# chaeyeongyun/VQ_SEG

Hardware: AMD Instinct MI355X
Metric: train images/sec @512x512 vqreptunet1x1 K=512 (higher is better)
Workload: dtype bf16; 1 GPU; CPS training iteration (2 x vqreptunet1x1, ResNet-50 encoder, K=[0,0,512,512,512], v1 recipe: 6 forwards + 4 backwards + 2 Adam steps) on 512x512x3 images -- BASELINE configs[2] (the metric's configuration): vqreptunet1x1 512x512, K = 512; labelled_per_gpu=32, unlabelled_per_gpu=32, parallelism=dp1, collectives=none (one process), conv_dtype=bf16

## Files before the change

include/vqseg.h:

```cpp
#ifndef VQSEG_H
#define VQSEG_H

#include <stddef.h>
#include <stdint.h>

#ifdef __cplusplus
extern "C" {
#endif

#define VQSEG_ABI_VERSION 1

#define VQSEG_EINVAL  (-1)
#define VQSEG_ENOSPC  (-2)
#define VQSEG_ENODEV  (-3)

int         vqseg_abi_version(void);
const char* vqseg_last_error(void);
const char* vqseg_kernel_name(const char* entry_point);

int vqseg_set_option(const char* key, int value);

int vqseg_profile_begin(int capacity);
int vqseg_profile_collect(int max_records, int64_t* n_rows_host, int* channels_host,
                          int* n_codes_host, float* ms_host,
// ... 52 lines not shown
int vqseg_kmeans_finalize_f32(const float* sums, const int64_t* counts, float* means,
                              int channels, int n_codes, void* stream);


int vqseg_vq_code_sums(int bf16, const void* x, const int64_t* idx, int64_t n_rows, int channels, int n_codes,
                       float* sums, int64_t* counts, void* workspace, size_t workspace_bytes, void* stream);
int vqseg_vq_ema_update_f32(float* cluster_size, float* embed_avg, float* codebook, const float* sums,
                            const int64_t* counts, int channels, int n_codes, float decay, float eps, float* scratch,
                            void* stream);
int vqseg_vq_revive_candidates(int bf16, const void* x, int64_t n_rows, int channels, int n_codes, uint64_t seed,
                               const int64_t* counter, int rank, int world, float* cand, float* ok, void* stream);
int vqseg_vq_ema_update_revive_f32(float* cluster_size, float* embed_avg, float* codebook, const float* sums,
                                   const int64_t* counts, int channels, int n_codes, float decay, float eps, float* scratch,
                                   const float* cand, const float* ok, float threshold, int64_t* counter, int64_t* revived,
                                   void* stream);


size_t vqseg_conv_packed_elems(int cout, int cin, int kh, int kw, int transpose_flip);
int vqseg_conv_pack_weights_f32(const float* w, int cout, int cin, int kh, int kw, int transpose_flip,
                                void* hi, void* lo, void* stream);

int64_t vqseg_conv_stat_slots(int64_t m_rows, int cout);
int vqseg_conv2d_f(const void* x, const void* x2, int c1, const void* w_hi, const void* w_lo, void* y,
                   float* stat_partial, int n, int h, int w, int cin, int cout, int kh, int kw, int stride,
                   int pad, int reflect, int up, int ho, int wo, int precise, void* stream);

int vqseg_conv2d_affine_f(const void* x, const void* x2, int c1, const void* w_hi, const void* w_lo,
                          const float* scale, const float* shift, const void* res, int relu, void* y,
                          int n, int h, int w, int cin, int cout, int kh, int kw, int stride, int pad, int reflect,
                          int ho, int wo, int precise, void* stream);
int vqseg_conv2d_affine_bits_f(const void* x, const void* w_hi, const float* scale, const float* shift, const void* res,
                               const unsigned char* res_bits, void* y, int n, int h, int w, int cin, int cout, int kh, int kw,
                               int pad, int ho, int wo, void* stream);

size_t vqseg_conv2d_wgrad_workspace_bytes(int n, int h, int w, int cin, int ho, int wo, int cout, int kh, int kw);
int vqseg_conv2d_wgrad_f(const void* gy, const void* x, const void* x2, int c1, int n, int h, int w, int cin,
                         int ho, int wo, int cout, int kh, int kw, int stride, int pad, int reflect, int precise,
                         int cin_out, int im2col, int accumulate, void* workspace, size_t workspace_bytes, float* gw,
                         void* stream);
int vqseg_conv2d_wgrad2_f(const void* gy, const void* x, const void* x2, int n, const void* gy_b, const void* x_b, const void* x2_b,
                          int n_b, int c1, int h, int w, int cin, int ho, int wo, int cout, int kh, int kw, int stride, int pad,
                          int reflect, int precise, int cin_out, int im2col, int accumulate, void* workspace, size_t workspace_bytes,
                          float* gw, void* stream);

int vqseg_bn_sync_ints(int c);
int vqseg_bn_finalize_f(float* partial, int64_t m_rows, int c, const float* gamma, const float* beta,
                        float* run_mean, float* run_var, float momentum, float eps, int training,
                        float* scale, float* shift, float* save_mean, float* save_invstd,
                        int64_t* num_batches_tracked , int* sync, void* stream);
int vqseg_bn_apply_f(int bf16, const void* y, const void* res, const float* scale, const float* shift,
                     int64_t m_rows, int c, int relu, void* out, void* stream);
size_t vqseg_bn_backward_workspace_floats(int64_t m_rows, int c);
int vqseg_bn_backward_f(int bf16, const void* g_out, const void* out, const void* y, const float* mean,
                        const float* invstd, const float* gamma, const float* fwd_scale, const float* fwd_shift,
                        int64_t m_rows, int c, int relu, int training, int accumulate,
                        float* workspace, float* dgamma, float* dbeta, void* g_y, void* g_res, int* sync, void* stream);
int vqseg_bn_apply_bits_f(const void* y, const void* res, const float* scale, const float* shift, int64_t m_rows, int c,
                          void* out, unsigned char* bits, void* stream);
int vqseg_bn_backward_bits_f(const void* g_out, const unsigned char* bits, const void* y, const float* mean,
                             const float* invstd, const float* gamma, int64_t m_rows, int c, int training, int accumulate,
                             float* workspace, float* dgamma, float* dbeta, void* g_y, void* g_res, int* sync, void* stream);

int vqseg_maxpool3x3s2_f(int bf16, int backward, const void* x, const void* g, int n, int h, int w, int c,
                         void* out, unsigned char* idx, void* stream);

int vqseg_bilinear_f(int bf16, int backward, const void* src, int n, int h, int w, int c, int ho, int wo,
// ... 123 lines not shown
```

vq_seg_amd/_hip.py:

```python
from __future__ import annotations

import ctypes
import os
from ctypes import c_char_p, c_double, c_float, c_int, c_int64, c_size_t, c_void_p
from typing import Optional, Tuple

import numpy as np
import torch

_HERE = os.path.dirname(os.path.abspath(__file__))
LIB_PATH = os.environ.get("VQSEG_LIB") or os.path.join(_HERE, "libvqseg_hip.so")

SYMBOLS = {
    "vqseg_abi_version": (c_int, []),
    "vqseg_last_error": (c_char_p, []),
    "vqseg_kernel_name": (c_char_p, [c_char_p]),
    "vqseg_set_option": (c_int, [c_char_p, c_int]),
    "vqseg_profile_begin": (c_int, [c_int]),
    "vqseg_profile_collect": (c_int, [c_int, c_void_p, c_void_p, c_void_p, c_void_p, c_void_p]),
    "vqseg_conv_profile_begin": (c_int, [c_int]),
    "vqseg_conv_profile_collect": (c_int, [c_int, c_void_p, c_void_p, c_void_p, c_void_p]),
    "vqseg_vq_workspace_bytes": (c_size_t, [c_int64, c_int, c_int]),
    "vqseg_vq_filter_counter_offset": (c_size_t, [c_int64, c_int, c_int]),
    "vqseg_vq_tiles_per_wave": (c_int, [c_int, c_void_p, c_void_p]),
    "vqseg_vq_forward_f32": (c_int, [c_void_p, c_void_p, c_void_p, c_int64, c_int, c_int, c_int, c_float, c_void_p,
                                     c_void_p, c_void_p, c_void_p, c_void_p, c_void_p, c_size_t, c_void_p]),
    "vqseg_vq_forward_bf16": (c_int, [c_void_p, c_void_p, c_void_p, c_int64, c_int, c_int, c_int, c_float, c_void_p,
                                      c_void_p, c_void_p, c_void_p, c_void_p, c_void_p, c_size_t, c_void_p]),
    "vqseg_vq_forward_group": (c_int, [c_int, c_int] + [c_void_p] * 6 + [c_int, c_void_p] + [c_void_p] * 6 + [c_void_p]),
    "vqseg_vq_backward_bf16": (c_int, [c_void_p, c_void_p, c_void_p, c_void_p, c_void_p, c_int64, c_int, c_float, c_void_p, c_void_p]),
    "vqseg_vq_assign_f32": (c_int, [c_void_p, c_void_p, c_void_p, c_int64, c_int, c_int, c_void_p, c_void_p, c_void_p,
                                    c_size_t, c_void_p]),
    "vqseg_vq_assign_bf16": (c_int, [c_void_p, c_void_p, c_void_p, c_int64, c_int, c_int, c_void_p, c_void_p, c_void_p,
                                     c_size_t, c_void_p]),
    "vqseg_vq_prepared_bytes": (c_size_t, [c_int, c_int]),
    "vqseg_vq_prepare_f32": (c_int, [c_void_p, c_int, c_int, c_void_p, c_size_t, c_void_p]),
    "vqseg_vq_backward_f32": (c_int, [c_void_p, c_void_p, c_void_p, c_void_p, c_int64, c_int, c_float, c_void_p,
                                      c_void_p]),
    "vqseg_kmeans_workspace_bytes": (c_size_t, [c_int64, c_int, c_int]),
    "vqseg_kmeans_f32": (c_int, [c_void_p, c_void_p, c_void_p, c_int64, c_int, c_int, c_int, c_void_p, c_size_t,
                                 c_void_p]),
    "vqseg_kmeans_accumulate_f32": (c_int, [c_void_p, c_void_p, c_int64, c_int, c_int, c_void_p, c_void_p, c_void_p,
                                            c_size_t, c_void_p]),
    "vqseg_kmeans_finalize_f32": (c_int, [c_void_p, c_void_p, c_void_p, c_int, c_int, c_void_p]),
    "vqseg_vq_code_sums": (c_int, [c_int, c_void_p, c_void_p, c_int64, c_int, c_int, c_void_p, c_void_p, c_void_p, c_size_t, c_void_p]),
    "vqseg_vq_ema_update_f32": (c_int, [c_void_p, c_void_p, c_void_p, c_void_p, c_void_p, c_int, c_int, c_float, c_float, c_void_p,
                                        c_void_p]),
    "vqseg_vq_revive_candidates": (c_int, [c_int, c_void_p, c_int64, c_int, c_int, ctypes.c_uint64, c_void_p, c_int, c_int, c_void_p, c_void_p,
                                           c_void_p]),
    "vqseg_vq_ema_update_revive_f32": (c_int, [c_void_p, c_void_p, c_void_p, c_void_p, c_void_p, c_int, c_int, c_float, c_float, c_void_p,
                                               c_void_p, c_void_p, c_float, c_void_p, c_void_p, c_void_p]),
    "vqseg_conv_packed_elems": (c_size_t, [c_int] * 5),
    "vqseg_conv_pack_weights_f32": (c_int, [c_void_p] + [c_int] * 5 + [c_void_p, c_void_p, c_void_p]),
    "vqseg_conv_stat_slots": (c_int64, [c_int64, c_int]),
    "vqseg_conv2d_f": (c_int, [c_void_p, c_void_p, c_int, c_void_p, c_void_p, c_void_p, c_void_p] + [c_int] * 14 + [c_void_p]),
    "vqseg_conv2d_affine_f": (c_int, [c_void_p, c_void_p, c_int, c_void_p, c_void_p, c_void_p, c_void_p, c_void_p, c_int, c_void_p] +
                              [c_int] * 13 + [c_void_p]),
    "vqseg_conv2d_wgrad_workspace_bytes": (c_size_t, [c_int] * 9),
    "vqseg_conv2d_wgrad_f": (c_int, [c_void_p, c_void_p, c_void_p] + [c_int] * 17 + [c_void_p, c_size_t, c_void_p, c_void_p]),
    "vqseg_conv2d_wgrad2_f": (c_int, [c_void_p, c_void_p, c_void_p, c_int, c_void_p, c_void_p, c_void_p, c_int] + [c_int] * 16 +
                              [c_void_p, c_size_t, c_void_p, c_void_p]),
    "vqseg_bn_sync_ints": (c_int, [c_int]),
    "vqseg_bn_finalize_f": (c_int, [c_void_p, c_int64, c_int, c_void_p, c_void_p, c_void_p, c_void_p, c_float, c_float, c_int,
                                   c_void_p, c_void_p, c_void_p, c_void_p, c_void_p, c_void_p, c_void_p]),
    "vqseg_bn_apply_f": (c_int, [c_int, c_void_p, c_void_p, c_void_p, c_void_p, c_int64, c_int, c_int, c_void_p, c_void_p]),
    "vqseg_bn_backward_workspace_floats": (c_size_t, [c_int64, c_int]),
    "vqseg_bn_backward_f": (c_int, [c_int] + [c_void_p] * 8 + [c_int64, c_int, c_int, c_int, c_int] + [c_void_p] * 7),
    "vqseg_conv2d_affine_bits_f": (c_int, [c_void_p] * 7 + [c_int] * 10 + [c_void_p]),
    "vqseg_bn_apply_bits_f": (c_int, [c_void_p] * 4 + [c_int64, c_int, c_void_p, c_void_p, c_void_p]),
    "vqseg_bn_backward_bits_f": (c_int, [c_void_p] * 6 + [c_int64, c_int, c_int, c_int] + [c_void_p] * 7),
    "vqseg_maxpool3x3s2_f": (c_int, [c_int, c_int, c_void_p, c_void_p, c_int, c_int, c_int, c_int, c_void_p, c_void_p, c_void_p]),
    "vqseg_bilinear_f": (c_int, [c_int, c_int, c_void_p] + [c_int] * 7 + [c_void_p, c_void_p]),
    "vqseg_head1x1_forward_f": (c_int, [c_int, c_void_p, c_void_p, c_int64, c_int, c_int, c_void_p, c_void_p]),
    "vqseg_head1x1_backward_workspace_floats": (c_size_t, [c_int64, c_int, c_int]),
    "vqseg_head1x1_backward_f": (c_int, [c_int, c_void_p, c_void_p, c_void_p, c_int64, c_int, c_int, c_void_p, c_void_p,
                                        c_void_p, c_void_p]),
    "vqseg_proto_loss_workspace_bytes": (c_size_t, [c_int64, c_int, c_int]),
    "vqseg_proto_loss_forward_f": (c_int, [c_int, c_void_p, c_void_p, c_void_p, c_void_p, c_void_p, c_int64, c_int, c_int, c_int,
                                           c_float, c_float, c_int, c_void_p, c_size_t, c_void_p, c_void_p]),
    "vqseg_proto_loss_backward_f": (c_int, [c_int, c_void_p, c_void_p, c_void_p, c_void_p, c_void_p, c_int64, c_int, c_int, c_int,
                                            c_float, c_float, c_int, c_void_p, c_void_p, c_void_p, c_void_p, c_size_t, c_void_p]),
    "vqseg_dice_workspace_bytes": (c_size_t, [c_int, c_int, c_int64]),
    "vqseg_dice_sums_forward_f": (c_int, [c_void_p, c_int64, c_int64, c_int64, c_void_p, c_int, c_int, c_int64, c_int64, c_void_p, c_size_t,
                                          c_void_p, c_void_p, c_void_p]),
    "vqseg_dice_sums_backward_f": (c_int, [c_void_p, c_int64, c_int64, c_int64, c_void_p, c_int, c_int, c_int64, c_int64, c_void_p,
                                           c_void_p, c_void_p, c_void_p]),
    "vqseg_dice_ce_sums_forward_f": (c_int, [c_void_p, c_int64, c_int64, c_int64, c_void_p, c_int, c_int, c_int64, c_int64, c_void_p,
                                             c_size_t, c_void_p, c_void_p, c_void_p, c_void_p]),
    "vqseg_dice_ce_sums_backward_f": (c_int, [c_void_p, c_int64, c_int64, c_int64, c_void_p, c_int, c_int, c_int64, c_int64, c_void_p,
                                              c_void_p, c_void_p, c_void_p, c_void_p]),
# ... 482 lines not shown
```

vq_seg_amd/csrc/conv_kernels.h:

```cpp
#pragma once
#include <hip/hip_runtime.h>
#include <stddef.h>
#include <stdint.h>

namespace vqseg {

struct ConvArgs {
    const void* x;
    const void* x2;
    int C1;
    const unsigned short* w_hi;
    const unsigned short* w_lo;
    void* y;
    float* stat_partial;
    int N, H, W, Cin, Ho, Wo, Cout, KH, KW, stride, pad, reflect, up;
    const float* ep_scale;
    const float* ep_shift;
    const void* ep_res;
    int ep_relu;
    int pair_chunks = 0, pair_tiles = 0;
    int out_s3 = 0;
    int s3_in = 0, s3_cs1 = 0, s3_cs2 = 0;
    int pad_w = -1;
    int omap = 0, omap_h = 0, omap_w = 0, omap_ph = 0, omap_pw = 0;
// ... 21 lines not shown
    int per_tap_only;
    const void* gy_b = nullptr;
    const void* x_b = nullptr;
    const void* x2_b = nullptr;
    int Na = 0;
    int xcd_slabs = 0;
};

hipError_t launch_conv(const ConvArgs& a, int precise, hipStream_t st);
long dgrad_s2_fold_rows(int N, int H, int W, int reflect);
hipError_t launch_dgrad_s2_fold(const void* gy, const unsigned short* w_hi, void* gx, int N, int Ho, int Wo, int Cout, int Cin, int H, int W,
                                int reflect, hipStream_t st);
hipError_t launch_stem7_fused(const float* x, const unsigned short* w_img, void* y, float* stat_partial, const float* ep_scale, const float* ep_shift,
                              int relu, int N, int H, int W, int reflect, int s3, hipStream_t st);
hipError_t conv_profile_begin(int capacity);
void conv_profile_release();
int conv_profile_collect(int max_records, double* flops, int* kind, float* ms, int* shape);
int conv_set_option(const char* key, int value);
int wgrad_slabs(const WgradArgs& a, int precise);
int wgrad_slabs_max(const WgradArgs& a);
hipError_t launch_wgrad(const WgradArgs& a, int precise, int slabs, int* final_layout, hipStream_t st);
hipError_t launch_wgrad_reduce(const float* partial, int slabs, int Cout, int Cin, int Cin_out, int KH, int KW, int im2col, int accumulate,
                               float* gw, hipStream_t st);
size_t packed_elems(int Cout, int Cin, int KH, int KW, int transpose_flip);
hipError_t launch_pack_weights(const float* w, int Cout, int Cin, int KH, int KW, int transpose_flip, unsigned short* hi,
                               unsigned short* lo, hipStream_t st);
hipError_t launch_pack_all(const float* w, int Cout, int Cin, int K, int C1, unsigned short* fwd, unsigned short* tr, unsigned short* s3,
                           hipStream_t st);
hipError_t launch_pack_weights_s2(const float* w, int Cout, int Cin, int K, unsigned short* hi, unsigned short* lo, hipStream_t st);
hipError_t launch_dgrad_s2(const void* gy, const unsigned short* w_hi, const unsigned short* w_lo, void* gx, int N, int Ho, int Wo,
                           int Cout, int Cin, int K, int OH, int OW, int precise, int accumulate, hipStream_t st);
hipError_t launch_reflect_ring(const void* gy, const unsigned short* t_hi, void* ring, int N, int H, int W, int Cgy, int Cgx, hipStream_t st);
hipError_t launch_pack_weights_s3(const float* w, int Cout, int Cin, int C1, int KH, int KW, unsigned short* out, hipStream_t st);

}
```

vq_seg_amd/csrc/nn_abi.hip:

```cpp
#include <hip/hip_runtime.h>
#include <stdarg.h>
#include <stdio.h>
#include <string.h>

#include "../../include/vqseg.h"
#include "conv_kernels.h"
#include "vq_kernels.h"
#include "nn_kernels.h"
#include "loss_kernels.h"
#include <math.h>

extern "C" int vqseg_set_error(int code, const char* msg);

namespace {
int bad(const char* msg) { return vqseg_set_error(VQSEG_EINVAL, msg); }
int hipfail(hipError_t e, const char* where) {
    char buf[256];
    snprintf(buf, sizeof(buf), "%s: %s", where, hipGetErrorString(e));
    return vqseg_set_error((int)e, buf);
}
bool a16(const void* p) { return (reinterpret_cast<uintptr_t>(p) & 15u) == 0; }

int conv_rows_per_slot(int cout) { return cout >= 64 ? 64 : 32; }
}
// ... 55 lines not shown
                          int kw, int stride, int pad, int reflect, int ho, int wo, int precise, void* stream) {
    if (!scale || !shift) return bad("conv2d_affine: null scale / shift");
    if (res && !a16(res)) return bad("conv2d_affine: pointers must be 16-byte aligned");
    if (precise == 2) {
        if (cin % 32 || cout % 8 || c1 % 32 || c1 <= 0 || c1 > cin) return bad("conv2d_affine (split-3): needs Cin, C1 % 32 == 0 and Cout % 8 == 0");
        if (!x || !w_hi || !y || (c1 < cin && !x2)) return bad("conv2d: null pointer");
        if (n <= 0 || h <= 0 || w <= 0 || ho <= 0 || wo <= 0 || kh <= 0 || kw <= 0 || stride <= 0) return bad("conv2d: non-positive dimension");
        if (!a16(x) || !a16(x2) || !a16(w_hi) || !a16(y)) return bad("conv2d: pointers must be 16-byte aligned");
        if (reflect && (pad >= h || pad >= w)) return bad("conv2d: reflect padding needs pad < size");
        vqseg::ConvArgs a;
        a.x = x; a.x2 = x2; a.C1 = 3 * c1;
        a.w_hi = static_cast<const unsigned short*>(w_hi); a.w_lo = nullptr;
        a.y = y; a.stat_partial = nullptr;
        a.N = n; a.H = h; a.W = w; a.Cin = 3 * cin; a.Ho = ho; a.Wo = wo; a.Cout = cout; a.KH = kh; a.KW = kw;
        a.stride = stride; a.pad = pad; a.reflect = reflect; a.up = 1;
        a.ep_scale = scale; a.ep_shift = shift; a.ep_res = res; a.ep_relu = relu;
        a.out_s3 = 1;
        a.s3_in = 1; a.s3_cs1 = c1; a.s3_cs2 = cin - c1;
        hipError_t e = vqseg::launch_conv(a, 0, static_cast<hipStream_t>(stream));
        return e == hipSuccess ? 0 : hipfail(e, "conv kernel (split-3)");
    }
    return conv2d_impl(x, x2, c1, w_hi, w_lo, y, nullptr, scale, shift, res, relu, n, h, w, cin, cout, kh, kw, stride, pad, reflect, 1,
                       ho, wo, precise, stream);
}

int vqseg_conv2d_affine_bits_f(const void* x, const void* w_hi, const float* scale, const float* shift, const void* res,
                               const unsigned char* res_bits, void* y, int n, int h, int w, int cin, int cout, int kh, int kw, int pad,
                               int ho, int wo, void* stream) {
    if (!scale || !shift || !res || !res_bits) return bad("conv2d_affine_bits: null pointer");
    if (!a16(res)) return bad("conv2d_affine_bits: pointers must be 16-byte aligned");
    if (cout % 8) return bad("conv2d_affine_bits: Cout must be a multiple of 8");
    return conv2d_impl(x, nullptr, cin, w_hi, nullptr, y, nullptr, scale, shift, res, 0, n, h, w, cin, cout, kh, kw, 1, pad, 0, 1, ho, wo, 0,
                       stream, res_bits);
}

int vqseg_conv_profile_begin(int capacity) {
    if (capacity <= 0 || capacity > (1 << 20)) return bad("conv_profile_begin: capacity out of range");
    hipError_t e = vqseg::conv_profile_begin(capacity);
    return e == hipSuccess ? 0 : hipfail(e, "conv_profile_begin");
}

int vqseg_conv_profile_collect(int max_records, double* flops_host, int* kind_host, float* ms_host, int* shape_host) {
    if (max_records <= 0 || !flops_host || !kind_host || !ms_host) return bad("conv_profile_collect: bad argument");
    return vqseg::conv_profile_collect(max_records, flops_host, kind_host, ms_host, shape_host);
}

int vqseg_set_option(const char* key, int value) {
    if (!key || value < 0) return bad("set_option: null key or negative value");
    int prev = vqseg::conv_set_option(key, value);
    if (prev < 0) prev = vqseg::vq_set_option(key, value);
    if (prev < 0) prev = vqseg::nn_set_option(key, value);
    return prev < 0 ? bad("set_option: unknown key") : prev;
}

size_t vqseg_conv2d_wgrad_workspace_bytes(int n, int h, int w, int cin, int ho, int wo, int cout, int kh, int kw) {
    if (n <= 0 || cin <= 0 || cout <= 0) return 0;
    vqseg::WgradArgs a{};
    a.N = n; a.H = h; a.W = w; a.Cin = cin; a.Ho = ho; a.Wo = wo; a.Cout = cout; a.KH = kh; a.KW = kw;
    return (size_t)vqseg::wgrad_slabs_max(a) * cout * kh * kw * cin * sizeof(float);
}

int vqseg_conv2d_wgrad2_f(const void* gy, const void* x, const void* x2, int n, const void* gy_b, const void* x_b, const void* x2_b,
                          int n_b, int c1, int h, int w, int cin, int ho, int wo, int cout, int kh, int kw, int stride, int pad,
                          int reflect, int precise, int cin_out, int im2col, int accumulate, void* workspace, size_t workspace_bytes,
                          float* gw, void* stream) {
    if (!gy || !x || !workspace || !gw) return bad("conv2d_wgrad: null pointer");
// ... 495 lines not shown
```

vq_seg_amd/models/networks/modified_vqunet/net.py:

```python
import torch
from torch import nn

from .... import nnf
from ....vector_quantizer import make_vq_module, Identity as _IdentityVQ, quantize_group as _quantize_group
from ...encoders import make_encoder
from ...modules.prototype import ReliablePrototypeLoss, ReliablePrototypeLossv2
from ..unet.decoder import UnetDecoder
from ..unet.net import _to_device_layout


class _Upsampling(nn.Module):

    def __init__(self, scale_factor):
        super().__init__()
        self.scale_factor = scale_factor

    def forward(self, x):
        return nnf.upsample_bilinear(x, scale_factor=self.scale_factor, align_corners=True)


class _Head1x1(nn.Conv2d):
    def forward(self, x):
        return nnf.head_conv1x1(x, self.weight)

# ... 7 lines not shown
        super().__init__()
        self.encoder = make_encoder(encoder_name, in_channels, depth, weights=encoder_weights, padding_mode="reflect")
        enc_ch = self.encoder.out_channels()
        self.codebook = make_vq_module(vq_cfg, enc_ch, depth)
        if decoder_channels is None:
            decoder_channels = [c // 2 for c in enc_ch[1:]][::-1]
        self.decoder = UnetDecoder(enc_ch, decoder_channels)
        self.segmentation_head = _Head1x1(decoder_channels[-1], num_classes, 1, bias=False)
        self.prototype_loss = self._proto_cls(num_classes, decoder_channels[-1], margin=margin, scale=scale, init=pt_init,
                                              use_feature=use_feature)
        self.device = None
        self.upsampling = _Upsampling(upsampling) if upsampling > 1 else nn.Identity()

    def encode(self, x):
        if self.device is None:
            self.device = x.device
        with nnf.s3_scope(not self.training and not torch.is_grad_enabled()):
            feats = self.encoder(_to_device_layout(x))[1:]
        if len(feats) != len(self.codebook):
            raise NotImplementedError
        return feats

    def quantize(self, feats):
        loss = torch.zeros(1, device=feats[0].device)
        usage = []
        levels = [i for i, vq in enumerate(self.codebook) if not isinstance(vq, _IdentityVQ)]
        for i in levels:
            if isinstance(feats[i], nnf.S3):
                feats[i] = feats[i].float()
        grouped = _quantize_group([self.codebook[i] for i in levels], [feats[i] for i in levels]) if nnf.py_opt("py_vq_group", 1) else None
        grouped = dict(zip(levels, grouped)) if grouped is not None else {}
        for i, vq in enumerate(self.codebook):
            quantize, _idx, commitment, dead = grouped[i] if i in grouped else vq(feats[i])
            feats[i] = quantize
            if commitment is not None:
                loss = loss + commitment
            if dead is not None:
                usage.append(dead.detach())
        return feats, loss / len(feats), usage

    def decode(self, feats):
        decoder_out = self.decoder(*feats)
        if self.training:
            nnf.fanin_tag(decoder_out)
        return decoder_out, self.segmentation_head(decoder_out)

    def _trunk(self, x):
        feats, loss, usage = self.quantize(self.encode(x))
        decoder_out, logits = self.decode(feats)
        return decoder_out, logits, loss, usage

    async_code_usage = False

    def _usage_to_host(self, usage, like):
        if not usage:
            return torch.tensor([])
        stacked = torch.stack(usage)
        if not (self.async_code_usage and stacked.is_cuda):
            return stacked.cpu()
        ring = self.__dict__.setdefault("_usage_ring", [])
        if len(ring) < 8:
            ring.append(torch.empty(stacked.shape, dtype=stacked.dtype, pin_memory=True))
        buf = ring[self.__dict__.setdefault("_usage_i", 0) % len(ring)]
        self.__dict__["_usage_i"] += 1
        buf.copy_(stacked, non_blocking=True)
        return buf

# ... 43 lines not shown
```

vq_seg_amd/models/networks/unet/decoder.py:

```python
from torch import nn

from .... import nnf as _nnf


class ConvBNReLU(nn.Sequential):

    def __init__(self, in_channels: int, out_channels: int, kernel_size: int = 3):
        super().__init__(nn.Conv2d(in_channels, out_channels, kernel_size, padding=int((kernel_size - 1) / 2), bias=False),
                         nn.BatchNorm2d(out_channels), nn.ReLU())

    def forward(self, x, x2=None):
        return _nnf.conv_bn_act(x, self[0], self[1], relu=True, x2=x2)


def conv_bn_relu(in_channels: int, out_channels: int, kernel_size: int = 3):
    return ConvBNReLU(in_channels, out_channels, kernel_size)


def double_conv_block(in_channels: int, out_channels: int, kernel_size: int = 3):
    return nn.Sequential(conv_bn_relu(in_channels, out_channels, kernel_size),
                         conv_bn_relu(out_channels, out_channels, kernel_size))


class UnetDecoder(nn.Module):
    def __init__(self, encoder_channels, decoder_channels):
        super().__init__()
        enc = list(encoder_channels[1:])[::-1]
        blocks, prev = [], 0
        for i, out_ch in enumerate(decoder_channels):
            blocks.append(double_conv_block(enc[i] + prev, out_ch))
            prev = out_ch
        self.blocks = nn.ModuleList(blocks)

    def forward(self, *features):
        dt = features[0].dtype
        feats = [_nnf.cast_act(f, dt) for f in features[::-1]]
        if any(isinstance(f, _nnf.S3) for f in feats):
            feats = [_nnf.to_s3(f) for f in feats]
        out = self.blocks[0][1](self.blocks[0][0](feats[0]))
        for i in range(1, len(self.blocks)):
            up = _nnf.upsample_bilinear(out, size=feats[i].shape[-2:], align_corners=False)
            out = self.blocks[i][1](self.blocks[i][0](up, feats[i]))
        return out
```

vq_seg_amd/nnf.py:

```python
from __future__ import annotations

from collections import namedtuple
import contextlib
import ctypes
from typing import Optional
import weakref

import torch

from . import _hip
from ._hip import lib
from ._wcache import cache_of as _cache_of, invalidate as invalidate_weight_caches


def _rows(x: torch.Tensor) -> torch.Tensor:
    v = x.permute(0, 2, 3, 1)
    return v if v.is_contiguous() else v.contiguous()


def _nchw(rows: torch.Tensor) -> torch.Tensor:
    return rows.permute(0, 3, 1, 2)


def _is_bf16(t: torch.Tensor) -> int:
# ... 525 lines not shown
            w2[:, :kh * kw * cin, 0, 0] = w.permute(0, 2, 3, 1).reshape(cout, kh * kw * cin)
            w = w2
        w = w if w.is_contiguous() else w.contiguous()
        cout, cin, kh, kw = w.shape
        out = torch.empty(cout * kh * kw * 3 * cin, dtype=torch.int16, device=w.device)
        _launch("vqseg_conv_pack_weights_s3_f32", w.device, _f32(w, "weight", cout * cin * kh * kw), cout, cin, c1, kh, kw,
                _w16(out, "split-3 image", cout * kh * kw * 3 * cin))
        cache[k] = out
    return cache[k]


def _conv_bn_act_s3(x: "S3", x2, residual, conv, bn, relu, kernel_1x1_cols: int = 0) -> "S3":
    n, h, w, _ = x.rows.shape
    c1 = x.c
    x2s = to_s3(x2) if x2 is not None else None
    cin = c1 + (x2s.c if x2s is not None else 0)
    cout = conv.weight.shape[0]
    if kernel_1x1_cols:
        kh = kw = 1
        stride, pad, reflect = 1, 0, False
    else:
        kh, kw = conv.weight.shape[2], conv.weight.shape[3]
        stride, pad = conv.stride[0], conv.padding[0]
        reflect = conv.padding_mode == "reflect" and pad > 0
    g = ConvGeom(n, h, w, c1, cin, cout, kh, kw, stride, pad, reflect, _out_size(h, kh, stride, pad), _out_size(w, kw, stride, pad))
    wimg = _s3_weights(conv.weight, c1, kernel_1x1_cols)
    res = to_s3(residual) if residual is not None else None
    coef = _bn_finalize(None, g.m, cout, bn.weight, bn.bias, bn, False, x.rows.device)
    out = _conv_affine(x.rows, x2s.rows if x2s is not None else None, wimg, None, coef[0], coef[1], res.rows if res is not None else None,
                       relu, g, 2)
    return S3(out, cout)


def _residual_rows(residual, dtype):
    rr = _rows(residual) if residual is not None else None
    if rr is not None and rr.dtype != dtype:
        raise _hip.HipLibraryError("residual dtype differs from the activation dtype")
    return rr


def _forward_eval(xr, x2r, residual, w_hi, w_lo, gamma, beta, bn, relu, g: ConvGeom, bf, stem):
    rr = _residual_rows(residual, xr.dtype)
    coef = _bn_finalize(None, g.m, g.cout, gamma, beta, bn, False, xr.device)
    if stem is not None and stem.is_fused:
        return _stem7_conv(xr, w_hi, None, coef, relu, stem, g.cout)
    return _conv_affine(xr, x2r, w_hi, w_lo, coef[0], coef[1], rr, relu, g, int(not bf))


class _ConvBNAct(torch.autograd.Function):
    @staticmethod
    def forward(ctx, x, x2, residual, weight, gamma, beta, bn, stride, pad, reflect, relu, stem, fuse_eval=False,
                link_in=None, link_out=None, link_x=None, fan_x=None, fan_x2=None):
        xr = _rows(x)
        x2r = _rows(x2) if x2 is not None else None
        bf = _is_bf16(xr)
        n, h, w, c1 = xr.shape
        fused = stem is not None and stem.is_fused
        stem_x = None
        if fused:
            stem_x, _STEM_X_ARG[0] = _STEM_X_ARG[0], None
            (h, w, c1), bf = stem.fused, 1
        cin = c1 + (x2r.shape[3] if x2r is not None else 0)
        cout = weight.shape[0]
        kh, kw = (1, 1) if stem is not None else (weight.shape[2], weight.shape[3])
        g = ConvGeom(n, h, w, c1, cin, cout, kh, kw, stride, pad, bool(reflect), _out_size(h, kh, stride, pad), _out_size(w, kw, stride, pad))
        training = bool(bn.training)
        if fused:
            w_hi, w_lo = _stem_weights_fused(weight, False), None
        elif stem is not None:
            w_hi, w_lo = _stem_weights(weight, not bf, cin)
        else:
            w_hi, w_lo = packed_weights(weight, not bf, False)
        if bn.momentum is None:
            raise NotImplementedError("BatchNorm2d(momentum=None) (cumulative average) is not used by the path")
        if fuse_eval and not training:
            return _nchw(_forward_eval(xr, x2r, residual, w_hi, w_lo, gamma, beta, bn, relu, g, bf, stem))
        stat = torch.empty(_stat_elems(g.m, cout), dtype=torch.float32, device=xr.device) if training else None
        y = _stem7_conv(xr, w_hi, stat, None, False, stem, cout) if fused else _conv_raw(xr, x2r, w_hi, w_lo, stat, g)
        coef = _bn_finalize(stat, g.m, cout, gamma, beta, bn, training, xr.device)
        rr = _residual_rows(residual, y.dtype)
        if rr is not None and relu and bf and cout % 8 == 0 and training and any(ctx.needs_input_grad) and py_opt("py_bn_bits", 1):
            out, bits = _bn_apply_bits(y, rr, coef, g.m, cout)
        else:
            out, bits = _bn_apply(y, rr, coef, g.m, cout, relu), None
        ctx.mask_bits = bits is not None
        if link_in is not None:
            link_in.takes_bits = bool(bf and x2r is None and stride == 1 and not reflect and cin % 8 == 0 and py_opt("py_gres_bits", 1))
        ctx.save_for_backward(xr, x2r, y, bits if bits is not None else out, coef, weight, gamma)
        ctx.stem_x = stem_x
        ctx.params = (weight, gamma, beta)
        ctx.bn = bn
        ctx.links = (link_in, link_out, link_x)
        ctx.fans = (fan_x, fan_x2)
        ctx.geom, ctx.stem = g, stem
        ctx.relu, ctx.training, ctx.has_res = bool(relu), training, residual is not None
        return _nchw(out)

    @staticmethod
    def backward(ctx, g_out):
        xr, x2r, y, out, coef, weight, gamma = ctx.saved_tensors
        g, stem = ctx.geom, ctx.stem
        if stem is not None and stem.is_fused:
            img = xr
            xr = _shared_stem_patches(ctx.stem_x if ctx.stem_x is not None else img,
                                      (torch.bfloat16, stem.kh, stem.kw, stem.stride, stem.pad, stem.reflect),
                                      lambda: _stem_patches(img, torch.bfloat16, stem.kh, stem.kw, stem.stride, stem.pad, stem.reflect, g.ho, g.wo, g.cin))
        g_y, g_res, dgamma, dbeta = _bn_backward_step(ctx, g_out, y, out, coef, gamma)
        gw = _wgrad_step(ctx, g_y, xr, x2r, weight)
        gx = gx2 = None
        if (ctx.needs_input_grad[0] or ctx.needs_input_grad[1]) and stem is None:
            gx, gx2 = _dgrad_step(ctx, g_y, x2r, weight)
# ... 163 lines not shown
        if not (g2.dtype == x2r.dtype and _fanin_deposit(fan_x2, g2)):
            gx2 = _nchw(g2)
    return gx, gx2


def _s2_weights(weight, precise):
    cache = _cache_of(weight)
    k = ("s2", precise)
    if k not in cache:
        w = weight.detach()
        w = w if w.is_contiguous() else w.contiguous()
        cout, cin, kh, _kw = w.shape
        nel = lib().vqseg_conv_packed_s2_elems(cout, cin, kh)
        hi = torch.empty(nel, dtype=torch.int16, device=w.device)
        lo = torch.empty(nel, dtype=torch.int16, device=w.device) if precise else None
        _launch("vqseg_conv_pack_weights_s2_f32", w.device, _f32(w, "weight", cout * cin * kh * kh), cout, cin, kh,
                _w16(hi, "parity-class image", nel), _w16(lo, "parity-class image (lo)", nel))
        cache[k] = (hi, lo)
    return cache[k]


def _stem_weights(weight, precise, kp):
    cache = _cache_of(weight)
    k = ("stem", precise, kp)
    if k not in cache:
        cout, cin, kh, kw = weight.shape
        w2 = torch.zeros(cout, kp, 1, 1, dtype=torch.float32, device=weight.device)
        w2[:, :kh * kw * cin, 0, 0] = weight.detach().permute(0, 2, 3, 1).reshape(cout, kh * kw * cin)
        cache[k] = packed_weights(w2, precise, False)
        cache[("stem_keepalive", precise, kp)] = w2
    return cache[k]


def conv_bn_act(x, conv, bn, training=None, relu=True, residual=None, x2=None, link_in=None, link_out=None, link_x=None, absorb_fanin=False):
    if conv.bias is not None:
        raise NotImplementedError("conv_bn_act: the reference's fused blocks have no conv bias")
    if isinstance(x, S3) or isinstance(x2, S3) or isinstance(residual, S3):
        c1 = x.shape[1]
        c2 = x2.shape[1] if x2 is not None else 0
        s3_ok = c1 % 32 == 0 and c2 % 32 == 0 and conv.weight.shape[0] % 8 == 0
        if not bn.training and not torch.is_grad_enabled() and s3_ok:
            return _conv_bn_act_s3(to_s3(x), x2, residual, conv, bn, relu)
        x, x2, residual = from_s3(x), (from_s3(x2) if x2 is not None else None), (from_s3(residual) if residual is not None else None)
    if not x.is_cuda:
        raise _hip.HipLibraryError(f"the HIP path needs 'cuda' (ROCm) tensors, got {x.device}; there is no CPU fallback")
    pad = conv.padding[0]
    _sink_use(conv.weight, bn.weight, bn.bias)
    return _ConvBNAct.apply(x, x2, residual, conv.weight, bn.weight, bn.bias, bn, conv.stride[0], pad,
                            conv.padding_mode == "reflect" and pad > 0, relu, None, not bn.training and not torch.is_grad_enabled(),
                            link_in, link_out, link_x, _fanin_of(x) if absorb_fanin else None, _fanin_of(x2))


_STEM_SHARE = None


def stem_share_begin():
    global _STEM_SHARE
    _STEM_SHARE = []


def stem_share_end():
    global _STEM_SHARE
    _STEM_SHARE = None


def _shared_stem_patches(x, cfg, make):
    if _STEM_SHARE is None:
        return make()
    cur = torch.cuda.current_stream(x.device)
    for ref, ver, key, patches, ev, st in _STEM_SHARE:
        if ref() is x and ver == x._version and key == cfg:
            if st != cur:
                cur.wait_event(ev)
                patches.record_stream(cur)
            return patches
    patches = make()
    ev = torch.cuda.Event()
    ev.record(cur)
    _STEM_SHARE.append((weakref.ref(x), x._version, cfg, patches, ev, cur))
    return patches


_STEM_X_ARG = [None]
# ... 616 lines not shown
```

Baseline: 441.6 images/sec.

## Replace decoder's first 3x3 conv on VQ codes with precomputed code-tap table gathers

When the decoder's first conv input is a vector-quantized tensor, each pixel holds one of K codebook vectors. A 3x3 conv is then a sum of 9 gathered rows from a table of size 9*K*Cout, built from the codebook times each weight tap. New HIP kernels build this table with MFMA and do the gather-sum, writing BN partial statistics in the training path and fusing the BN affine in the eval path. This removes the dense conv FLOPs for that layer. The cost is table construction plus index-driven gathers, and the table cache has to be invalidated correctly when the weights or codebook change.

```diff
diff --git a/include/vqseg.h b/include/vqseg.h
--- a/include/vqseg.h
+++ b/include/vqseg.h
@@ -108,6 +108,11 @@
 int vqseg_conv2d_affine_bits_f(const void* x, const void* w_hi, const float* scale, const float* shift, const void* res,
                                const unsigned char* res_bits, void* y, int n, int h, int w, int cin, int cout, int kh, int kw,
                                int pad, int ho, int wo, void* stream);
+
+int vqseg_code_tap_table_f(int form, const void* w, const float* codebook, int n_codes, int c1, int cin, int cout, float* table,
+                           void* stream);
+int vqseg_code_tap_sum_f(int mode, const float* table, const int64_t* idx, int n_codes, int n, int h, int w, int cout, void* out,
+                         float* stat_partial, const float* scale, const float* shift, int relu, void* stream);
 
 size_t vqseg_conv2d_wgrad_workspace_bytes(int n, int h, int w, int cin, int ho, int wo, int cout, int kh, int kw);
 int vqseg_conv2d_wgrad_f(const void* gy, const void* x, const void* x2, int c1, int n, int h, int w, int cin,
diff --git a/vq_seg_amd/_hip.py b/vq_seg_amd/_hip.py
--- a/vq_seg_amd/_hip.py
+++ b/vq_seg_amd/_hip.py
@@ -56,6 +56,8 @@
     "vqseg_conv2d_f": (c_int, [c_void_p, c_void_p, c_int, c_void_p, c_void_p, c_void_p, c_void_p] + [c_int] * 14 + [c_void_p]),
     "vqseg_conv2d_affine_f": (c_int, [c_void_p, c_void_p, c_int, c_void_p, c_void_p, c_void_p, c_void_p, c_void_p, c_int, c_void_p] +
                               [c_int] * 13 + [c_void_p]),
+    "vqseg_code_tap_table_f": (c_int, [c_int, c_void_p, c_void_p, c_int, c_int, c_int, c_int, c_void_p, c_void_p]),
+    "vqseg_code_tap_sum_f": (c_int, [c_int, c_void_p, c_void_p] + [c_int] * 5 + [c_void_p] * 4 + [c_int, c_void_p]),
     "vqseg_conv2d_wgrad_workspace_bytes": (c_size_t, [c_int] * 9),
     "vqseg_conv2d_wgrad_f": (c_int, [c_void_p, c_void_p, c_void_p] + [c_int] * 17 + [c_void_p, c_size_t, c_void_p, c_void_p]),
     "vqseg_conv2d_wgrad2_f": (c_int, [c_void_p, c_void_p, c_void_p, c_int, c_void_p, c_void_p, c_void_p, c_int] + [c_int] * 16 +
diff --git a/vq_seg_amd/csrc/code_taps.hip b/vq_seg_amd/csrc/code_taps.hip
--- /dev/null
+++ b/vq_seg_amd/csrc/code_taps.hip
@@ -0,0 +1,245 @@
+#include <hip/hip_runtime.h>
+
+#include "conv_device.h"
+
+namespace vqseg {
+
+__global__ __launch_bounds__(256) void code_tap_table_bf16_kernel(const unsigned short* __restrict__ wimg, const float* __restrict__ cb, int K,
+                                                                  int C1, int C2, int cin_p, int Cout, float* __restrict__ T) {
+    const int r = threadIdx.x & 31, h = (threadIdx.x >> 5) & 1;
+    const int co0 = blockIdx.x * 64, k0 = (blockIdx.y * 4 + (threadIdx.x >> 6)) * 64, t = blockIdx.z;
+    if (k0 >= K) return;
+    f32x16 acc[2][2];
+#pragma unroll
+    for (int a = 0; a < 2; ++a)
+#pragma unroll
+        for (int b = 0; b < 2; ++b)
+#pragma unroll
+            for (int i = 0; i < 16; ++i) acc[a][b][i] = 0.0f;
+    const float* ap[2];
+    const unsigned short* bp[2];
+#pragma unroll
+    for (int a = 0; a < 2; ++a) {
+        const int k = k0 + a * 32 + r;
+        ap[a] = cb + (long)(k < K ? k : K - 1) * C2;
+        const int co = co0 + a * 32 + r;
+        bp[a] = wimg + ((long)(co < Cout ? co : Cout - 1) * 9 + t) * cin_p + C1;
+    }
+    for (int c0 = 0; c0 < C2; c0 += 64) {
+#pragma unroll
+        for (int j = 0; j < 4; ++j) {
+            const int c = c0 + h * 32 + j * 8;
+            bf16x8 af[2], bf[2];
+#pragma unroll
+            for (int a = 0; a < 2; ++a) {
+#pragma unroll
+                for (int e = 0; e < 8; ++e) af[a][e] = (__bf16)0.0f, bf[a][e] = (__bf16)0.0f;
+                if (c < C2) {
+                    const f32x4 lo = *reinterpret_cast<const f32x4*>(ap[a] + c), hi = *reinterpret_cast<const f32x4*>(ap[a] + c + 4);
+#pragma unroll
+                    for (int e = 0; e < 4; ++e) af[a][e] = (__bf16)lo[e], af[a][4 + e] = (__bf16)hi[e];
+                    bf[a] = __builtin_bit_cast(bf16x8, *reinterpret_cast<const u32x4*>(bp[a] + c));
+                }
+            }
+#pragma unroll
+            for (int a = 0; a < 2; ++a)
+#pragma unroll
+                for (int b = 0; b < 2; ++b) acc[a][b] = __builtin_amdgcn_mfma_f32_32x32x16_bf16(af[a], bf[b], acc[a][b], 0, 0, 0);
+        }
+    }
+#pragma unroll
+    for (int a = 0; a < 2; ++a)
+#pragma unroll
+        for (int b = 0; b < 2; ++b) {
+            const int co = co0 + b * 32 + r;
+#pragma unroll
+            for (int i = 0; i < 16; ++i) {
+                const int k = k0 + a * 32 + (i & 3) + 8 * (i >> 2) + 4 * h;
+                if (k < K && co < Cout) T[((long)t * K + k) * Cout + co] = acc[a][b][i];
+            }
+        }
+}
+
+__global__ __launch_bounds__(256) void code_tap_table_f32_kernel(const float* __restrict__ w, const float* __restrict__ cb, int K, int C1, int C2,
+                                                                 int Cin, int Cout, float* __restrict__ T) {
+    const int r = threadIdx.x & 31, h = (threadIdx.x >> 5) & 1;
+    const int co0 = blockIdx.x * 32, k0 = (blockIdx.y * 4 + (threadIdx.x >> 6)) * 64, kh = blockIdx.z;
+    if (k0 >= K) return;
+    f32x16 acc[2][3];
+#pragma unroll
+    for (int a = 0; a < 2; ++a)
+#pragma unroll
+        for (int q = 0; q < 3; ++q)
+#pragma unroll
+            for (int i = 0; i < 16; ++i) acc[a][q][i] = 0.0f;
+    const float* ap[2];
+#pragma unroll
+    for (int a = 0; a < 2; ++a) ap[a] = cb + (long)(k0 + a * 32 + r < K ? k0 + a * 32 + r : K - 1) * C2;
+    const float* bp = w + ((long)(co0 + r < Cout ? co0 + r : Cout - 1) * Cin + C1) * 9 + kh * 3;
+    f32x4 a0, a1, na0, na1;
+    float b[4][3], nb[4][3];
+    auto load = [&](int c0, f32x4& x0, f32x4& x1, float (&y)[4][3]) {
+        const int c = c0 + h * 4;
+        x0 = *reinterpret_cast<const f32x4*>(ap[0] + c);
+        x1 = *reinterpret_cast<const f32x4*>(ap[1] + c);
+#pragma unroll
+        for (int j = 0; j < 4; ++j)
+#pragma unroll
+            for (int q = 0; q < 3; ++q) y[j][q] = bp[(long)(c + j) * 9 + q];
+    };
+    load(0, a0, a1, b);
+    for (int c0 = 0; c0 < C2; c0 += 8) {
+        if (c0 + 8 < C2) load(c0 + 8, na0, na1, nb);
+#pragma unroll
+        for (int j = 0; j < 4; ++j)
+#pragma unroll
+            for (int q = 0; q < 3; ++q) {
+                acc[0][q] = __builtin_amdgcn_mfma_f32_32x32x2f32(a0[j], b[j][q], acc[0][q], 0, 0, 0);
+                acc[1][q] = __builtin_amdgcn_mfma_f32_32x32x2f32(a1[j], b[j][q], acc[1][q], 0, 0, 0);
+            }
+        a0 = na0, a1 = na1;
+#pragma unroll
+        for (int j = 0; j < 4; ++j)
+#pragma unroll
+            for (int q = 0; q < 3; ++q) b[j][q] = nb[j][q];
+    }
+    const int co = co0 + r;
+#pragma unroll
+    for (int a = 0; a < 2; ++a)
+#pragma unroll
+        for (int q = 0; q < 3; ++q)
+#pragma unroll
+            for (int i = 0; i < 16; ++i) {
+                const int k = k0 + a * 32 + (i & 3) + 8 * (i >> 2) + 4 * h;
+                if (k < K && co < Cout) T[((long)(kh * 3 + q) * K + k) * Cout + co] = acc[a][q][i];
+            }
+}
+
+hipError_t launch_code_tap_table(int form, const void* w, const float* codebook, int K, int C1, int Cin, int Cout, float* table, hipStream_t st) {
+    const int C2 = Cin - C1;
+    const unsigned groups = (unsigned)((K + 255) / 256);
+    if (form == 0) {
+        const int cin_p = (Cin + 31) / 32 * 32;
+        hipLaunchKernelGGL(code_tap_table_bf16_kernel, dim3((Cout + 63) / 64, groups, 9), dim3(256), 0, st, static_cast<const unsigned short*>(w),
+                           codebook, K, C1, C2, cin_p, Cout, table);
+    } else {
+        hipLaunchKernelGGL(code_tap_table_f32_kernel, dim3((Cout + 31) / 32, groups, 3), dim3(256), 0, st, static_cast<const float*>(w), codebook, K,
+                           C1, C2, Cin, Cout, table);
+    }
+    return hipGetLastError();
+}
+
+constexpr int TAP_RS = 8, TAP_CHUNK = 128, TAP_MAX_GRID = 2048;
+
+template <int MODE, int RPS>
+__global__ __launch_bounds__(256) void code_tap_sum_kernel(const float* __restrict__ T, const long long* __restrict__ idx, int K, int H, int W,
+                                                           int Cout, long M, long n_slots, void* __restrict__ out, float* __restrict__ stat,
+                                                           const float* __restrict__ scale, const float* __restrict__ shift, int relu) {
+    constexpr int RPT = RPS / TAP_RS;
+    __shared__ float red[TAP_RS][TAP_CHUNK];
+    const int cg = threadIdx.x & 31, rs = threadIdx.x >> 5;
+    const int co = blockIdx.y * TAP_CHUNK + cg * 4;
+    const bool cok = co < Cout;
+    const unsigned hw = (unsigned)(H * W);
+    f32x4 sc = {1.f, 1.f, 1.f, 1.f}, sh = {0.f, 0.f, 0.f, 0.f};
+    if (MODE == 2 && cok) sc = *reinterpret_cast<const f32x4*>(scale + co), sh = *reinterpret_cast<const f32x4*>(shift + co);
+    for (long slot = blockIdx.x; slot < n_slots; slot += gridDim.x) {
+        f32x4 v[RPT];
+#pragma unroll
+        for (int j = 0; j < RPT; ++j) {
+            const long m = slot * RPS + rs + j * TAP_RS;
+            f32x4 a = {0.f, 0.f, 0.f, 0.f};
+            if (m < M && cok) {
+                const unsigned um = (unsigned)m, n = um / hw, rem = um - n * hw;
+                const int oh = (int)(rem / (unsigned)W), ow = (int)(rem - (unsigned)oh * (unsigned)W);
+#pragma unroll
+                for (int t = 0; t < 9; ++t) {
+                    const int ih = oh + t / 3 - 1, iw = ow + t % 3 - 1;
+                    if (ih < 0 || ih >= H || iw < 0 || iw >= W) continue;
+                    long long k = idx[(long)n * hw + (long)ih * W + iw];
+                    k = k < 0 ? 0 : (k >= K ? K - 1 : k);
+                    const f32x4 tv = *reinterpret_cast<const f32x4*>(T + ((long)t * K + k) * Cout + co);
+                    a += tv;
+                }
+                if (MODE == 0) *reinterpret_cast<f32x4*>(static_cast<float*>(out) + m * Cout + co) = a;
+                if (MODE == 1) {
+                    u32x2 o = {pack2(a[0], a[1]), pack2(a[2], a[3])};
+                    *reinterpret_cast<u32x2*>(static_cast<unsigned short*>(out) + m * Cout + co) = o;
+                }
+                if (MODE == 2) {
+                    float y[4];
+#pragma unroll
+                    for (int e = 0; e < 4; ++e) {
+                        y[e] = __builtin_fmaf(a[e], sc[e], sh[e]);
+                        if (relu && !(y[e] > 0.0f)) y[e] = 0.0f;
+                    }
+                    u32x2 oh_ = {pack2(y[0], y[1]), pack2(y[2], y[3])};
+                    u32x2 ol_ = {pack2(y[0] - bf16_round(y[0]), y[1] - bf16_round(y[1])), pack2(y[2] - bf16_round(y[2]), y[3] - bf16_round(y[3]))};
+                    unsigned short* yp = static_cast<unsigned short*>(out) + m * 2 * Cout + co;
+                    *reinterpret_cast<u32x2*>(yp) = oh_;
+                    *reinterpret_cast<u32x2*>(yp + Cout) = ol_;
+                }
+            }
+            v[j] = a;
+        }
+        if (MODE == 1 && stat) {
+            long cnt_l = M - slot * RPS;
+            const float cnt = (float)(cnt_l > RPS ? RPS : cnt_l);
+            f32x4 s = {0.f, 0.f, 0.f, 0.f};
+#pragma unroll
+            for (int j = 0; j < RPT; ++j)
+                if (slot * RPS + rs + j * TAP_RS < M) s += v[j];
+            *reinterpret_cast<f32x4*>(&red[rs][cg * 4]) = s;
+            __syncthreads();
+            f32x4 tot = *reinterpret_cast<const f32x4*>(&red[0][cg * 4]);
+#pragma unroll
+            for (int q = 1; q < TAP_RS; ++q) tot += *reinterpret_cast<const f32x4*>(&red[q][cg * 4]);
+            f32x4 mean, m2 = {0.f, 0.f, 0.f, 0.f};
+#pragma unroll
+            for (int e = 0; e < 4; ++e) mean[e] = tot[e] / cnt;
+#pragma unroll
+            for (int j = 0; j < RPT; ++j)
+                if (slot * RPS + rs + j * TAP_RS < M) {
+#pragma unroll
+                    for (int e = 0; e < 4; ++e) {
+                        const float d = v[j][e] - mean[e];
+                        m2[e] = __builtin_fmaf(d, d, m2[e]);
+                    }
+                }
+            __syncthreads();
+            *reinterpret_cast<f32x4*>(&red[rs][cg * 4]) = m2;
+            __syncthreads();
+            if (rs == 0 && cok) {
+                f32x4 mt = *reinterpret_cast<const f32x4*>(&red[0][cg * 4]);
+#pragma unroll
+                for (int q = 1; q < TAP_RS; ++q) mt += *reinterpret_cast<const f32x4*>(&red[q][cg * 4]);
+                *reinterpret_cast<f32x4*>(stat + (slot * 2 + 0) * Cout + co) = mean;
+                *reinterpret_cast<f32x4*>(stat + (slot * 2 + 1) * Cout + co) = mt;
+            }
+            __syncthreads();
+        }
+    }
+}
+
+template <int MODE>
+static void tap_sum_launch(int rps, dim3 grid, hipStream_t st, const float* T, const long long* idx, int K, int H, int W, int Cout, long M,
+                           long n_slots, void* out, float* stat, const float* scale, const float* shift, int relu) {
+    if (rps == 64)
+        hipLaunchKernelGGL((code_tap_sum_kernel<MODE, 64>), grid, dim3(256), 0, st, T, idx, K, H, W, Cout, M, n_slots, out, stat, scale, shift, relu);
+    else
+        hipLaunchKernelGGL((code_tap_sum_kernel<MODE, 32>), grid, dim3(256), 0, st, T, idx, K, H, W, Cout, M, n_slots, out, stat, scale, shift, relu);
+}
+
+hipError_t launch_code_tap_sum(int mode, const float* table, const long long* idx, int K, int N, int H, int W, int Cout, void* out, float* stat,
+                               const float* scale, const float* shift, int relu, hipStream_t st) {
+    const long M = (long)N * H * W;
+    const int rps = Cout >= 64 ? 64 : 32;
+    const long n_slots = (M + rps - 1) / rps;
+    const dim3 grid((unsigned)(n_slots < TAP_MAX_GRID ? n_slots : TAP_MAX_GRID), (unsigned)((Cout + TAP_CHUNK - 1) / TAP_CHUNK));
+    if (mode == 0) tap_sum_launch<0>(rps, grid, st, table, idx, K, H, W, Cout, M, n_slots, out, nullptr, nullptr, nullptr, 0);
+    else if (mode == 1) tap_sum_launch<1>(rps, grid, st, table, idx, K, H, W, Cout, M, n_slots, out, stat, nullptr, nullptr, 0);
+    else tap_sum_launch<2>(rps, grid, st, table, idx, K, H, W, Cout, M, n_slots, out, nullptr, scale, shift, relu);
+    return hipGetLastError();
+}
+
+}
diff --git a/vq_seg_amd/csrc/conv_kernels.h b/vq_seg_amd/csrc/conv_kernels.h
--- a/vq_seg_amd/csrc/conv_kernels.h
+++ b/vq_seg_amd/csrc/conv_kernels.h
@@ -77,5 +77,8 @@
                            int Cout, int Cin, int K, int OH, int OW, int precise, int accumulate, hipStream_t st);
 hipError_t launch_reflect_ring(const void* gy, const unsigned short* t_hi, void* ring, int N, int H, int W, int Cgy, int Cgx, hipStream_t st);
 hipError_t launch_pack_weights_s3(const float* w, int Cout, int Cin, int C1, int KH, int KW, unsigned short* out, hipStream_t st);
+hipError_t launch_code_tap_table(int form, const void* w, const float* codebook, int K, int C1, int Cin, int Cout, float* table, hipStream_t st);
+hipError_t launch_code_tap_sum(int mode, const float* table, const long long* idx, int K, int N, int H, int W, int Cout, void* out, float* stat,
+                               const float* scale, const float* shift, int relu, hipStream_t st);
 
 }
diff --git a/vq_seg_amd/csrc/nn_abi.hip b/vq_seg_amd/csrc/nn_abi.hip
--- a/vq_seg_amd/csrc/nn_abi.hip
+++ b/vq_seg_amd/csrc/nn_abi.hip
@@ -111,6 +111,30 @@
     if (cout % 8) return bad("conv2d_affine_bits: Cout must be a multiple of 8");
     return conv2d_impl(x, nullptr, cin, w_hi, nullptr, y, nullptr, scale, shift, res, 0, n, h, w, cin, cout, kh, kw, 1, pad, 0, 1, ho, wo, 0,
                        stream, res_bits);
+}
+
+int vqseg_code_tap_table_f(int form, const void* w, const float* codebook, int n_codes, int c1, int cin, int cout, float* table, void* stream) {
+    if (!w || !codebook || !table) return bad("code_tap_table: null pointer");
+    if (form != 0 && form != 1) return bad("code_tap_table: form must be 0 (bf16 image) or 1 (fp32 weight)");
+    if (n_codes <= 0 || cout <= 0 || c1 < 0 || c1 >= cin) return bad("code_tap_table: bad dimension");
+    if (c1 % 8 || (cin - c1) % 8) return bad("code_tap_table: C1 and Cin - C1 must be multiples of 8");
+    if (!a16(w) || !a16(codebook)) return bad("code_tap_table: pointers must be 16-byte aligned");
+    hipError_t e = vqseg::launch_code_tap_table(form, w, codebook, n_codes, c1, cin, cout, table, static_cast<hipStream_t>(stream));
+    return e == hipSuccess ? 0 : hipfail(e, "code_tap_table_kernel");
+}
+
+int vqseg_code_tap_sum_f(int mode, const float* table, const int64_t* idx, int n_codes, int n, int h, int w, int cout, void* out,
+                         float* stat_partial, const float* scale, const float* shift, int relu, void* stream) {
+    if (!table || !idx || !out) return bad("code_tap_sum: null pointer");
+    if (mode < 0 || mode > 2) return bad("code_tap_sum: mode must be 0, 1 or 2");
+    if (n_codes <= 0 || n <= 0 || h <= 0 || w <= 0 || cout <= 0) return bad("code_tap_sum: non-positive dimension");
+    if ((int64_t)n * h * w > 0x7fffffffLL) return bad("code_tap_sum: more than 2^31 - 1 pixels");
+    if (cout % 4) return bad("code_tap_sum: Cout must be a multiple of 4");
+    if (mode == 2 && (!scale || !shift)) return bad("code_tap_sum: null scale / shift");
+    if (!a16(table) || !a16(out) || !a16(stat_partial) || !a16(scale) || !a16(shift)) return bad("code_tap_sum: pointers must be 16-byte aligned");
+    hipError_t e = vqseg::launch_code_tap_sum(mode, table, reinterpret_cast<const long long*>(idx), n_codes, n, h, w, cout, out, stat_partial,
+                                              scale, shift, relu, static_cast<hipStream_t>(stream));
+    return e == hipSuccess ? 0 : hipfail(e, "code_tap_sum_kernel");
 }
 
 int vqseg_conv_profile_begin(int capacity) {
diff --git a/vq_seg_amd/models/networks/modified_vqunet/net.py b/vq_seg_amd/models/networks/modified_vqunet/net.py
--- a/vq_seg_amd/models/networks/modified_vqunet/net.py
+++ b/vq_seg_amd/models/networks/modified_vqunet/net.py
@@ -63,7 +63,7 @@
         grouped = dict(zip(levels, grouped)) if grouped is not None else {}
         for i, vq in enumerate(self.codebook):
             quantize, _idx, commitment, dead = grouped[i] if i in grouped else vq(feats[i])
-            feats[i] = quantize
+            feats[i] = quantize if _idx is None else nnf.code_tag(quantize, _idx, vq.codebook)
             if commitment is not None:
                 loss = loss + commitment
             if dead is not None:
diff --git a/vq_seg_amd/models/networks/unet/decoder.py b/vq_seg_amd/models/networks/unet/decoder.py
--- a/vq_seg_amd/models/networks/unet/decoder.py
+++ b/vq_seg_amd/models/networks/unet/decoder.py
@@ -1,3 +1,4 @@
+import torch
 from torch import nn
 
 from .... import nnf as _nnf
@@ -9,8 +10,8 @@
         super().__init__(nn.Conv2d(in_channels, out_channels, kernel_size, padding=int((kernel_size - 1) / 2), bias=False),
                          nn.BatchNorm2d(out_channels), nn.ReLU())
 
-    def forward(self, x, x2=None):
-        return _nnf.conv_bn_act(x, self[0], self[1], relu=True, x2=x2)
+    def forward(self, x, x2=None, codes=None, s3=False):
+        return _nnf.conv_bn_act(x, self[0], self[1], relu=True, x2=x2, codes=codes, s3=s3)
 
 
 def conv_bn_relu(in_channels: int, out_channels: int, kernel_size: int = 3):
@@ -34,10 +35,14 @@
 
     def forward(self, *features):
         dt = features[0].dtype
+        tag0 = _nnf.code_tag_of(features[-1])
         feats = [_nnf.cast_act(f, dt) for f in features[::-1]]
-        if any(isinstance(f, _nnf.S3) for f in feats):
-            feats = [_nnf.to_s3(f) for f in feats]
-        out = self.blocks[0][1](self.blocks[0][0](feats[0]))
+        s3 = any(isinstance(f, _nnf.S3) for f in feats)
+        kind = "s3" if s3 else ("bf16" if feats[0].dtype == torch.bfloat16 else None)
+        taps0 = _nnf.code_taps_plan(tag0, self.blocks[0][0][0], feats[0].shape, kind)
+        if s3:
+            feats = [f if (i == 0 and taps0) else _nnf.to_s3(f) for i, f in enumerate(feats)]
+        out = self.blocks[0][1](self.blocks[0][0](feats[0], codes=tag0 if taps0 else None, s3=s3))
         for i in range(1, len(self.blocks)):
             up = _nnf.upsample_bilinear(out, size=feats[i].shape[-2:], align_corners=False)
             out = self.blocks[i][1](self.blocks[i][0](up, feats[i]))
diff --git a/vq_seg_amd/nnf.py b/vq_seg_amd/nnf.py
--- a/vq_seg_amd/nnf.py
+++ b/vq_seg_amd/nnf.py
@@ -581,6 +581,73 @@
     return S3(out, cout)
 
 
+CODE_TAPS_MIN_RATIO = 4
+
+
+def code_tag(t, idx, codebook):
+    if torch.is_tensor(t) and torch.is_tensor(idx) and not codebook.ema_update:
+        t._vq_codes = (idx, codebook.embedding.weight)
+    return t
+
+
+def code_tag_of(t):
+    return getattr(t, "_vq_codes", None) if torch.is_tensor(t) else None
+
+
+def code_taps_plan(tag, conv, x_shape, kind: str) -> bool:
+    opt = py_opt("py_code_taps", 1)
+    if not opt or tag is None or kind not in ("bf16", "s3") or not py_opt("py_code_taps_" + kind, 1):
+        return False
+    idx, cb_w = tag
+    n, c, h, w = x_shape
+    cout, cin, kh, kw = conv.weight.shape
+    k, c2 = cb_w.shape
+    if not ((kh, kw) == (3, 3) and conv.stride == (1, 1) and conv.padding == (1, 1) and conv.dilation == (1, 1) and conv.groups == 1
+            and conv.padding_mode == "zeros" and conv.bias is None and cin == c2 == c and c2 % 8 == 0 and cout % 8 == 0
+            and tuple(idx.shape) == (n, h, w) and idx.dtype == torch.int64 and idx.is_cuda and idx.is_contiguous() and cb_w.is_cuda):
+        return False
+    return opt == 2 or n * h * w >= CODE_TAPS_MIN_RATIO * k
+
+
+def _code_tap_table(weight, cb_w, c1: int, form: int) -> torch.Tensor:
+    cout, cin = weight.shape[0], weight.shape[1]
+    k = cb_w.shape[0]
+    w_img = packed_weights(weight, False, False)[0] if form == 0 else None
+    cache, cb_cache = _cache_of(weight), _cache_of(cb_w)
+    ent = cache.get(("code_taps", form, c1))
+    if ent is None or ent[0] is not cb_cache:
+        table = torch.empty(9 * k * cout, dtype=torch.float32, device=weight.device)
+        if form == 0:
+            wp = _w16(w_img, "packed weights", _packed_elems(cout, 3, 3, cin))
+        else:
+            w = weight.detach()
+            wp = _f32(w if w.is_contiguous() else w.contiguous(), "weight", cout * cin * 9)
+        _launch("vqseg_code_tap_table_f", weight.device, form, wp, _f32(cb_w.detach(), "codebook", k * (cin - c1)), k, c1, cin, cout,
+                _f32(table, "tap table", 9 * k * cout))
+        cache[("code_taps", form, c1)] = ent = (cb_cache, table)
+    return ent[1]
+
+
+def _code_tap_sum(mode: int, table, idx, k: int, g: ConvGeom, stat=None, scale=None, shift=None, relu=False):
+    dtype, f = ((torch.float32, 1), (torch.bfloat16, 1), (torch.bfloat16, 2))[mode]
+    out = torch.empty((g.n, g.ho, g.wo, f * g.cout), dtype=dtype, device=table.device)
+    _launch("vqseg_code_tap_sum_f", table.device, mode, _f32(table, "tap table", 9 * k * g.cout),
+            _T(idx, "code indices", dtype=torch.int64, numel=g.n * g.h * g.w), k, g.n, g.h, g.w, g.cout,
+            _T(out, "tap sums", dtype=dtype, numel=g.m * g.cout * f), _f32(stat, "BN partials", _stat_elems(g.m, g.cout) if stat is not None else None),
+            _f32(scale, "scale", g.cout if scale is not None else None), _f32(shift, "shift", g.cout if shift is not None else None), int(relu))
+    return out
+
+
+def _conv_bn_act_codes_s3(codes, x_shape, conv, bn, relu) -> "S3":
+    idx, cb_w = codes
+    n, _, h, w = x_shape
+    cout, cin = conv.weight.shape[0], conv.weight.shape[1]
+    g = ConvGeom(n, h, w, cin, cin, cout, 3, 3, 1, 1, False, h, w)
+    coef = _bn_finalize(None, g.m, cout, bn.weight, bn.bias, bn, False, idx.device)
+    table = _code_tap_table(conv.weight, cb_w, 0, 1)
+    return S3(_code_tap_sum(2, table, idx, cb_w.shape[0], g, scale=coef[0], shift=coef[1], relu=relu), cout)
+
+
 def _residual_rows(residual, dtype):
     rr = _rows(residual) if residual is not None else None
     if rr is not None and rr.dtype != dtype:
@@ -599,7 +666,7 @@
 class _ConvBNAct(torch.autograd.Function):
     @staticmethod
     def forward(ctx, x, x2, residual, weight, gamma, beta, bn, stride, pad, reflect, relu, stem, fuse_eval=False,
-                link_in=None, link_out=None, link_x=None, fan_x=None, fan_x2=None):
+                link_in=None, link_out=None, link_x=None, fan_x=None, fan_x2=None, codes=None):
         xr = _rows(x)
         x2r = _rows(x2) if x2 is not None else None
         bf = _is_bf16(xr)
@@ -625,7 +692,10 @@
         if fuse_eval and not training:
             return _nchw(_forward_eval(xr, x2r, residual, w_hi, w_lo, gamma, beta, bn, relu, g, bf, stem))
         stat = torch.empty(_stat_elems(g.m, cout), dtype=torch.float32, device=xr.device) if training else None
-        y = _stem7_conv(xr, w_hi, stat, None, False, stem, cout) if fused else _conv_raw(xr, x2r, w_hi, w_lo, stat, g)
+        if codes is not None and bf and x2r is None and stem is None:
+            y = _code_tap_sum(1, _code_tap_table(weight, codes[1], 0, 0), codes[0], codes[1].shape[0], g, stat=stat)
+        else:
+            y = _stem7_conv(xr, w_hi, stat, None, False, stem, cout) if fused else _conv_raw(xr, x2r, w_hi, w_lo, stat, g)
         coef = _bn_finalize(stat, g.m, cout, gamma, beta, bn, training, xr.device)
         rr = _residual_rows(residual, y.dtype)
         if rr is not None and relu and bf and cout % 8 == 0 and training and any(ctx.needs_input_grad) and py_opt("py_bn_bits", 1):
@@ -855,9 +925,14 @@
     return cache[k]
 
 
-def conv_bn_act(x, conv, bn, training=None, relu=True, residual=None, x2=None, link_in=None, link_out=None, link_x=None, absorb_fanin=False):
+def conv_bn_act(x, conv, bn, training=None, relu=True, residual=None, x2=None, link_in=None, link_out=None, link_x=None, absorb_fanin=False,
+                codes=None, s3=False):
     if conv.bias is not None:
         raise NotImplementedError("conv_bn_act: the reference's fused blocks have no conv bias")
+    if codes is not None and s3:
+        if not bn.training and not torch.is_grad_enabled() and x2 is None and residual is None:
+            return _conv_bn_act_codes_s3(codes, x.shape, conv, bn, relu)
+        codes = None
     if isinstance(x, S3) or isinstance(x2, S3) or isinstance(residual, S3):
         c1 = x.shape[1]
         c2 = x2.shape[1] if x2 is not None else 0
@@ -871,7 +946,7 @@
     _sink_use(conv.weight, bn.weight, bn.bias)
     return _ConvBNAct.apply(x, x2, residual, conv.weight, bn.weight, bn.bias, bn, conv.stride[0], pad,
                             conv.padding_mode == "reflect" and pad > 0, relu, None, not bn.training and not torch.is_grad_enabled(),
-                            link_in, link_out, link_x, _fanin_of(x) if absorb_fanin else None, _fanin_of(x2))
+                            link_in, link_out, link_x, _fanin_of(x) if absorb_fanin else None, _fanin_of(x2), codes)
 
 
 _STEM_SHARE = None
```

After: 445.7 images/sec (median of 6 runs). Within noise of the previous version (+0.9%).
